# facebookresearch/brainmagick

Hardware: AMD Instinct MI355X
Metric: segments/s, 208-ch x 360-sample SimpleConv + ClipLoss training step (higher is better)
Workload: dtype f32 (fp32-accurate: operands split into 2 scaled f16 planes, 3 MFMA products, fp32 accumulate; same parity tolerances as exact fp32, see DESIGN.md §2); 1 GPU; cfg2: gwilliams2022-shaped MEG C=208 T=360, F=120 features, 27 subjects, clip_conv SimpleConv (8985590 params) + ClipLoss + Adam; batch_per_gpu=256, global_batch=256, negatives=local, parallelism=dp1, comm=none, rccl_world=1, candidate_gather=none, distinct_batches=8

## Files before the change

brainmagick_amd/csrc/core.hip:

```cpp
#include "bm_common.h"
#include <stdarg.h>
#include <stdlib.h>

thread_local char bm_err_buf[512] = {0};

int bm_set_error(int code, const char* fmt, ...) {
    va_list ap;
    va_start(ap, fmt);
    vsnprintf(bm_err_buf, sizeof(bm_err_buf), fmt, ap);
    va_end(ap);
    return code;
}

int bm_check_launch(const char* what) {
    hipError_t e = hipGetLastError();
    if (e != hipSuccess) return bm_set_error((int)e, "%s: launch failed: %s", what, hipGetErrorString(e));
    return BM_OK;
}

extern "C" const char* bm_last_error(void) { return bm_err_buf; }
extern "C" int bm_version(void) { return 108; }

extern "C" int bm_device_count(void) {
    int n = 0;
    hipError_t e = hipGetDeviceCount(&n);
    if (e != hipSuccess) { bm_set_error((int)e, "hipGetDeviceCount: %s", hipGetErrorString(e)); return -1; }
    return n;
}

__global__ __launch_bounds__(1024) void amax_finalize_kernel(const float* __restrict__ ws, int n, float* __restrict__ out) {
    __shared__ float sh[16];
    float m = 0.f;
    for (int i = threadIdx.x; i < n; i += 1024) m = fmaxf(m, ws[i]);
    m = bm_wave_max(m);
    if ((threadIdx.x & 63) == 0) sh[threadIdx.x >> 6] = m;
    __syncthreads();
    if (threadIdx.x < BM_AMAX_SHARDS) {
        float v = 0.f;
        if (threadIdx.x == 0)
            for (int w = 0; w < 16; ++w) v = fmaxf(v, sh[w]);
        out[threadIdx.x] = v;
    }
}

int bm_amax_finalize(const float* ws, int n, float* out, hipStream_t stream) {
    if (!out) return BM_OK;
    hipLaunchKernelGGL(amax_finalize_kernel, dim3(1), dim3(1024), 0, stream, ws, n, out);
    return bm_check_launch("amax_finalize");
}

__global__ __launch_bounds__(1024) void amax_finalize_rows_kernel(const float* __restrict__ ws, int C, int nsplit,
                                                                  float* __restrict__ out, float* __restrict__ rows_out,
                                                                  const double* __restrict__ sum_partial,
                                                                  float* __restrict__ sums_out) {
// ... 40 lines not shown
```

brainmagick_amd/csrc/norm_act.hip:

```cpp
#include <cstdlib>
#include "bm_common.h"

template <int VEC> struct Pack;
template <> struct Pack<1> {
    float v[1];
    __device__ static Pack ld(const float* p) { Pack r; r.v[0] = *p; return r; }
    __device__ void st(float* p) const { *p = v[0]; }
};
template <> struct Pack<4> {
    float v[4];
    __device__ static Pack ld(const float* p) {
        const float4 t = *reinterpret_cast<const float4*>(p);
        Pack r; r.v[0] = t.x; r.v[1] = t.y; r.v[2] = t.z; r.v[3] = t.w; return r;
    }
    __device__ void st(float* p) const { *reinterpret_cast<float4*>(p) = make_float4(v[0], v[1], v[2], v[3]); }
};

#define LAUNCH_VEC(vec4, kernel, grid, stream, ...)                                              \
    do {                                                                                         \
        if (vec4) hipLaunchKernelGGL(kernel<4>, grid, dim3(256), 0, stream, __VA_ARGS__);        \
        else hipLaunchKernelGGL(kernel<1>, grid, dim3(256), 0, stream, __VA_ARGS__);             \
    } while (0)
static int flat_blocks(long n) { return (int)((n + 255) / 256 > 16384 ? 16384 : (n + 255) / 256); }

// ... 577 lines not shown
    if (workspace_bytes < bm_channel_sum_workspace_bytes(B, C))
        return bm_set_error(BM_ERR_WORKSPACE, "channel_sum: workspace too small");
    hipStream_t s = (hipStream_t)stream;
    double* partial = (double*)workspace;
    LAUNCH_VEC(T % 4 == 0 && bstride % 4 == 0, channel_sum_kernel, dim3(C, nsplit), s, x, bstride, partial, B, C, T);
    hipLaunchKernelGGL(finalize_channel_sums_kernel, dim3(cdiv(C, 256)), dim3(256), 0, s, partial, out, C,
                       nsplit);
    return bm_check_launch("channel_sum");
}

__global__ __launch_bounds__(256) void time_sums_t_kernel(const float* __restrict__ x, float* __restrict__ out,
                                                          int B, int C, int T) {
    const long row = (long)blockIdx.x * 4 + (threadIdx.x >> 6);
    if (row >= (long)B * C) return;
    const int lane = threadIdx.x & 63;
    const float* p = x + row * T;
    float s = 0.f;
    for (int t = lane; t < T; t += 64) s += p[t];
    s = bm_wave_sum(s);
    if (lane == 0) {
        const int b = (int)(row / C), c = (int)(row - (long)b * C);
        out[(long)c * B + b] = s;
    }
}

extern "C" int bm_time_sums_t(const float* x, float* out, int B, int C, int T, void* stream) {
    BM_REQUIRE(x && out && B >= 0 && C > 0 && T > 0, "time_sums_t: bad arguments");
    if (B == 0) return BM_OK;
    hipLaunchKernelGGL(time_sums_t_kernel, dim3((unsigned)(((long)B * C + 3) / 4)), dim3(256), 0, (hipStream_t)stream,
                       x, out, B, C, T);
    return bm_check_launch("time_sums_t");
}

template <int VEC>
__global__ __launch_bounds__(256) void channel_stats_kernel(const float* __restrict__ x,
                                                            float* __restrict__ stats, int B, int C,
                                                            int T) {
    __shared__ double sh[4 * 2];
    const int c = blockIdx.x, split = blockIdx.y, nsplit = gridDim.y;
    const Slab sl(B, split, nsplit, T, VEC);
    float s = 0.f, s2 = 0.f;
    for (SlabWalk w(sl.TV, threadIdx.x, blockDim.x); w.bl < sl.nb; w.next()) {
        const int bl = w.bl, tv = w.tv;
        const Pack<VEC> v = Pack<VEC>::ld(x + ((long)(sl.b0 + bl) * C + c) * T + (long)tv * VEC);
#pragma unroll
        for (int i = 0; i < VEC; ++i) { s += v.v[i]; s2 += v.v[i] * v.v[i]; }
    }
    double acc[2] = {(double)s, (double)s2};
    block_sum<2>(acc, sh);
    if (threadIdx.x == 0) {
        stats[((long)split * C + c) * 2 + 0] = (float)acc[0];
        stats[((long)split * C + c) * 2 + 1] = (float)acc[1];
    }
}

extern "C" int bm_channel_stats_splits(int B) { return B >= 64 ? 16 : (B >= 8 ? 4 : 1); }

extern "C" int bm_channel_stats(const float* x, float* stats, int B, int C, int T, void* stream) {
    BM_REQUIRE(x && stats, "channel_stats: null pointer");
    const int nsplit = bm_channel_stats_splits(B);
    hipStream_t s = (hipStream_t)stream;
    LAUNCH_VEC(T % 4 == 0, channel_stats_kernel, dim3(C, nsplit), s, x, stats, B, C, T);
    return bm_check_launch("channel_stats");
}

template <int VEC>
// ... 109 lines not shown
```

brainmagick_amd/csrc/pack.hip:

```cpp
#include "bm_common.h"

__global__ void pack_weights_kernel(const float* __restrict__ src, float* __restrict__ dst, int G,
                                    int M, int Cin, int KS, long sg, long sm, long sc, long sj,
                                    int flip, int Mpad, int nchunk, const float* alpha_ptr) {
    const long total = (long)G * nchunk * KS * BM_BKC * Mpad;
    const float alpha = alpha_ptr ? *alpha_ptr : 1.f;
    for (long i = (long)blockIdx.x * blockDim.x + threadIdx.x; i < total;
         i += (long)gridDim.x * blockDim.x) {
        long r = i;
        const int m = (int)(r % Mpad); r /= Mpad;
        const int cc = (int)(r % BM_BKC); r /= BM_BKC;
        const int j = (int)(r % KS); r /= KS;
        const int chunk = (int)(r % nchunk);
        const int g = (int)(r / nchunk);
        const int c = chunk * BM_BKC + cc;
        float v = 0.f;
        if (m < M && c < Cin) {
            const int jj = flip ? KS - 1 - j : j;
            v = alpha * src[g * sg + m * sm + c * sc + jj * sj];
        }
        dst[i] = v;
    }
}

// ... 39 lines not shown
        int run = 0;
        for (int g = 0; g < G; ++g) { const int c = counts[g]; counts[g] = run; seg[g] = run; run += c; }
        counts[G] = run;
        seg[G] = run;
    }
    __syncthreads();
    for (int g = threadIdx.x; g < G; g += blockDim.x) {
        int pos = counts[g];
        const int end = counts[g + 1];
        for (int b0 = 0; b0 < B && pos < end; b0 += 8) {
            int v[8];
#pragma unroll
            for (int u = 0; u < 8; ++u) v[u] = b0 + u < B ? ids[b0 + u] : -1;
#pragma unroll
            for (int u = 0; u < 8; ++u)
                if (v[u] == g) order[pos++] = b0 + u;
        }
    }
}

#define BM_GROUP_MAX_INTS (64 * 1024 / 4)

extern "C" int bm_group_by_index(const long* idx, int B, int G, int* order, int* seg, int* err_flag,
                                 void* stream) {
    BM_REQUIRE(seg && ((idx && order) || B == 0), "group_by_index: null pointer");
    BM_REQUIRE(B >= 0 && G > 0, "group_by_index: bad dims B=%d G=%d", B, G);
    BM_REQUIRE((long)G + 1 + B <= BM_GROUP_MAX_INTS, "group_by_index: B + G + 1 = %ld ints of LDS exceed the %d of a "
               "launch (B=%d G=%d)", (long)G + 1 + B, BM_GROUP_MAX_INTS, B, G);
    hipLaunchKernelGGL(group_by_index_kernel, dim3(1), dim3(256), (size_t)(G + 1 + B) * sizeof(int),
                       (hipStream_t)stream, idx, B, G, order, seg, err_flag);
    return bm_check_launch("group_by_index");
}

__global__ void index_to_i32_kernel(const long* __restrict__ idx, int B, int G, int* __restrict__ out,
                                    int* __restrict__ err) {
    const int i = blockIdx.x * blockDim.x + threadIdx.x;
    if (i >= B) return;
    long v = idx[i];
    if (v < 0 || v >= G) {
        if (err) atomicExch(err, 1);
        v = 0;
    }
    out[i] = (int)v;
}

extern "C" int bm_index_to_i32(const long* idx, int B, int G, int* out, int* err_flag, void* stream) {
    BM_REQUIRE((idx && out) || B == 0, "index_to_i32: null pointer");
    BM_REQUIRE(B >= 0 && G > 0, "index_to_i32: bad dims B=%d G=%d", B, G);
    if (B == 0) return BM_OK;
    hipLaunchKernelGGL(index_to_i32_kernel, dim3((B + 255) / 256), dim3(256), 0, (hipStream_t)stream, idx, B,
                       G, out, err_flag);
    return bm_check_launch("index_to_i32");
}

__global__ void reduce_splits_kernel(const float* __restrict__ part, float* __restrict__ out, int G,
                                     int nsplit, int M, int Cn, int KS, long sg, long sm, long sc,
                                     long sj) {
    const long N = (long)Cn * KS;
    const long per = (long)M * N;
    const long total = (long)G * per;
    for (long i = (long)blockIdx.x * blockDim.x + threadIdx.x; i < total;
         i += (long)gridDim.x * blockDim.x) {
        const int g = (int)(i / per);
        const long r = i - (long)g * per;
        const int m = (int)(r / N);
        const int n = (int)(r - (long)m * N);
// ... 83 lines not shown
```

brainmagick_amd/functional.py:

```python

import torch

from . import hip_ops as H



ACT_CODES = {"none": H.ACT_NONE, "gelu": H.ACT_GELU, "relu": H.ACT_RELU, "leaky": H.ACT_LEAKY}


def _c(t: torch.Tensor) -> torch.Tensor:
    return t if t.is_contiguous() else t.contiguous()


_arange_cache = {}


def _arange_i32(n: int, device, repeat: int = 1) -> torch.Tensor:
    key = (n, repeat, device.type, device.index)
    t = _arange_cache.get(key)
    if t is None:
        if len(_arange_cache) > 64:
            _arange_cache.clear()
        t = torch.arange(n, dtype=torch.int32, device=device)
        if repeat != 1:
            t = t.repeat(repeat)
        if device.type == "cuda":
            torch.cuda.current_stream(device).synchronize()
        _arange_cache[key] = t
    return t


def _conv_weight_grads(dy, x, weight, KS, dil, transposed_weight):
    dst = H.grad_destination(weight)
    B, M, T = dy.shape
    Cin = x.shape[1]
    if transposed_weight:
        out = dst if dst is not None else torch.empty(weight.shape, device=dy.device, dtype=torch.float32)
        H.gemm_nt(x, dy, B, Cin, M, T, 1, 1, out=out.view(1, Cin, M, 1))
        return out.view(weight.shape) if dst is not None else out
    if dst is not None:
        H.gemm_nt(dy, x, B, M, Cin, T, KS, dil, out=dst.view(1, M, Cin, KS))
        return dst.view(weight.shape)
    return H.gemm_nt(dy, x, B, M, Cin, T, KS, dil).view(weight.shape)


def _layer_forward(x, weight, geom, res=None, **kw):
    dil, transposed, stride, pad = geom
    if pad is not None:
        assert res is None, "the strided family has no fused residual"
        KS = weight.shape[2]
        M = weight.shape[1] if transposed else weight.shape[0]
        Tout = H.conv_out_len(x.shape[2], KS, stride, dil, pad, transposed)
        wp = H.pack_strided_rows_second(weight) if transposed else H.pack_strided_rows_first(weight)
        return H.conv_strided(x, wp, M, Tout, KS, stride, dil, pad, transposed, **kw)
    assert stride == 1
    if transposed:
        Cin, M, KS = weight.shape
        assert KS == 1, "ConvTranspose1d is only supported with kernel 1 (simpleconv.py:189)"
# ... 185 lines not shown
        U, C, O, D = ctx.dims
        dout = _c(dout)
        B, _, T = meg.shape
        dheads = None
        if ctx.needs_input_grad[1]:
            order, seg = H.group_by_index(_c(layout_index.to(torch.int64)), U)
            dweights = H.gemm_nt(dout, meg, B, O, C, T, 1, 1, order=order, seg=seg, G=U).view(U, O, C)
            dscores = H.softmax_bwd(weights, dweights)
            wp = H.pack_weights(dscores, U, O, C, 1, O * C, C, 1, 0, shape=(D, 1))
            uidx = _arange_i32(U, meg.device)
            _, per_layout, _ = H.conv_nn(emb, wp, O, 1, 1, widx=uidx)
            if ctx.per_layout_heads:
                dheads = per_layout
            else:
                dheads = H.sum_over_batch(per_layout) if U > 1 else per_layout[0]
        dmeg = None
        if ctx.needs_input_grad[0]:
            wpt = H.pack_weights(weights, U, C, O, 1, O * C, 1, C, 0, shape=(T, 1))
            _, dmeg, _ = H.conv_nn(dout, wpt, C, 1, 1, widx=widx)
        return dmeg, dheads, None, None, None, None


class FusedFrontEndFn(torch.autograd.Function):

    @staticmethod
    def forward(ctx, meg, heads, w1, b1, ws, positions_u, layout_index, subjects, ban_center, ban_radius: float):
        meg, heads, w1, ws, positions_u = _c(meg), _c(heads), _c(w1), _c(ws), _c(positions_u)
        U, C, _ = positions_u.shape
        O, Dp = heads.shape
        L = w1.shape[0]
        S, _, D = ws.shape
        B, _, T = meg.shape
        dev = meg.device
        emb = H.fourier_emb(positions_u, Dp)
        seg_u = _arange_i32(U + 1, dev)
        scores = H.gemm_nt(heads, emb, U, O, C, Dp, a_strides=(0, Dp), x_strides=(C * Dp, Dp), seg=seg_u,
                           G=U).view(U, O, C)
        wm = H.masked_softmax(scores, positions_u, ban_center, ban_radius)
        _, p, _ = H.conv_nn(wm, H.pack_conv_fwd(w1), L, 1, 1)
        bcol = (b1 if b1 is not None else torch.zeros(L, device=dev)).view(1, L, 1).expand(U, L, 1)
        xp = torch.cat([p, bcol], dim=2).repeat_interleave(S, dim=0).contiguous()
        widx_p = _arange_i32(S, dev, repeat=U)
        _, wc, _ = H.conv_nn(xp, H.pack_weights(ws, S, D, L, 1, L * D, 1, D, 0), D, 1, 1, widx=widx_p)
        bias_c = wc[:, :, C].contiguous()
        pair = H.index_i32(_c(layout_index.to(torch.int64)), U) * S + H.index_i32(_c(subjects.to(torch.int64)), S)
        wpc = H.pack_weights(wc, U * S, D, C, 1, D * (C + 1), C + 1, 1, 0, shape=(T, 1))
        _, out, _ = H.conv_nn(meg, wpc, D, 1, 1, widx=pair, bias=bias_c, bias_gstride=D)
        ctx.save_for_backward(meg, emb, wm, xp, ws, w1, pair, widx_p, wc)
        ctx.dims = (U, C, O, Dp, L, S, D)
        ctx.has_b1 = b1 is not None
        return out

    @staticmethod
    def backward(ctx, dout):
        meg, emb, wm, xp, ws, w1, pair, widx_p, wc = ctx.saved_tensors
        U, C, O, Dp, L, S, D = ctx.dims
        dout = _c(dout)
        B, _, T = meg.shape
        dev = meg.device
        P = U * S
        order, seg = H.group_by_index(pair.to(torch.int64), P)
        gaug = torch.empty(P, D, C + 1, device=dev, dtype=torch.float32)
        H.gemm_nt(dout, meg, B, D, C, T, 1, 1, order=order, seg=seg, G=P, out=gaug,
                  out_strides=(D * (C + 1), C + 1, 1, 0))
        gaug[:, :, C] = H.segment_sum_cols(H.time_sums_t(dout), order, seg).t()
        seg_p = _arange_i32(P + 1, dev)
        dws = dw1 = db1 = dheads = None
        if ctx.needs_input_grad[4]:
            t1 = H.gemm_nt(xp, gaug, P, L, D, C + 1, seg=seg_p, G=P)
            dws = (H.sum_over_batch(t1.view(U, S * L * D)) if U > 1 else t1).view(S, L, D)
        _, a, _ = H.conv_nn(gaug, H.pack_weights(ws, S, L, D, 1, L * D, D, 1, 0), L, 1, 1, widx=widx_p)
        a_u = torch.stack([H.sum_over_batch(a[u * S:(u + 1) * S]) for u in range(U)])
        if ctx.has_b1 and ctx.needs_input_grad[3]:
            db1 = H.sum_over_batch(a_u[:, :, C].contiguous()) if U > 1 else a_u[0, :, C].contiguous()
        if ctx.needs_input_grad[2]:
            dw1 = H.gemm_nt(a_u, wm, U, L, O, C, 1, 1, a_strides=(L * (C + 1), C + 1),
                            x_strides=(O * C, C)).view(L, O, 1)
        if ctx.needs_input_grad[1]:
            _, dwm, _ = H.conv_nn(a_u, H.pack_conv_dgrad(w1), O, 1, 1)
            dscores = H.softmax_bwd(wm, dwm[:, :, :C].contiguous())
            wp = H.pack_weights(dscores, U, O, C, 1, O * C, C, 1, 0, shape=(Dp, 1))
            uidx = _arange_i32(U, dev)
            _, per_layout, _ = H.conv_nn(emb, wp, O, 1, 1, widx=uidx)
            dheads = H.sum_over_batch(per_layout) if U > 1 else per_layout[0]
        dmeg = None
        if ctx.needs_input_grad[0]:
            wpt = H.pack_weights(wc, P, C, D, 1, D * (C + 1), 1, C + 1, 0, shape=(T, 1))
            _, dmeg, _ = H.conv_nn(dout, wpt, C, 1, 1, widx=pair)
        return dmeg, dheads, dw1, db1, dws, None, None, None, None, None


_CLIP_BLOCK_BYTES = 0x3f000000


def _candidate_blocks(Bc: int, K: int):
    if Bc * K * 4 < _CLIP_BLOCK_BYTES:
        return [(0, Bc)]
    rows = max(1, _CLIP_BLOCK_BYTES // (K * 4))
    if rows >= 128:
        rows -= rows % 128
    return [(r0, min(rows, Bc - r0)) for r0 in range(0, Bc, rows)]


def _clip_raw_scores(estimate, candidate, B, Bc, K):
    blocks = _candidate_blocks(Bc, K)
    if len(blocks) == 1:
        return H.gemm_nt_partials(estimate, candidate, 1, B, Bc, K, (0, K), (0, K))
    raw = torch.empty(1, B, Bc, device=estimate.device, dtype=torch.float32)
    cand2 = candidate.view(Bc, K)
    for r0, rows in blocks:
        blk = H.share_amax(candidate, cand2[r0:r0 + rows])
        H.gemm_nt(estimate, blk, 1, B, rows, K, 1, 1, a_strides=(0, K), x_strides=(0, K),
                  out=raw.view(-1)[r0:], out_strides=(0, Bc, 1, 0))
    return raw


class ClipLossFn(torch.autograd.Function):

    @staticmethod
    def forward(ctx, estimate, candidate, target_offset: int = 0, col_valid=None, symmetric: bool = False,
# ... 180 lines not shown
```

brainmagick_amd/hip_ops.py:

```python
import ctypes
import typing as tp

import torch

from ._lib import lib, check, BmHipError

ACT_NONE, ACT_GELU, ACT_RELU, ACT_LEAKY = 0, 1, 2, 3
BKC = 16

import os as _os
DEFAULT_COMPUTE_DTYPE = "f16x2"
COMPUTE_DTYPES = ("f32", "f32x3", "f16x2")
_compute_dtype = _os.environ.get("BM_COMPUTE_DTYPE", DEFAULT_COMPUTE_DTYPE)
if _compute_dtype not in COMPUTE_DTYPES:
    raise ValueError(f"BM_COMPUTE_DTYPE must be one of {COMPUTE_DTYPES}, got {_compute_dtype!r}")


def set_compute_dtype(name: str):
    global _compute_dtype
    if name not in COMPUTE_DTYPES:
        raise ValueError(f"compute dtype must be one of {COMPUTE_DTYPES}, got {name!r}")
    _compute_dtype = name


# ... 653 lines not shown
                              _p(_opt(mean, "mean")), _p(_opt(invstd, "invstd")), int(bn_train),
                              _p(dy), _p(dgamma), _p(dbeta), _p(dbias), _p(ws), nbytes, B, C, T, act,
                              leak, *_slot_args(slot), _p(_row_amax_out(dy, slot)), _stream()), "bm_act_bn_bwd")
    return dy, dgamma, dbeta, dbias


def channel_sum(x: torch.Tensor) -> torch.Tensor:
    _req(x, "channel_sum.x")
    B, C, T = x.shape
    out = torch.empty(C, device=x.device, dtype=torch.float32)
    nbytes = lib().bm_channel_sum_workspace_bytes(B, C)
    ws = torch.empty(nbytes, device=x.device, dtype=torch.uint8)
    check(lib().bm_channel_sum(_p(x), C * T, _p(out), _p(ws), nbytes, B, C, T, _stream()),
          "bm_channel_sum")
    return out


def channel_stats(x: torch.Tensor) -> torch.Tensor:
    _req(x, "channel_stats.x")
    B, C, T = x.shape
    stats = torch.empty(lib().bm_channel_stats_splits(B), C, 2, device=x.device, dtype=torch.float32)
    check(lib().bm_channel_stats(_p(x), _p(stats), B, C, T, _stream()), "bm_channel_stats")
    return stats


def time_sums_t(x: torch.Tensor) -> torch.Tensor:
    _req(x, "time_sums_t.x")
    B, C, T = x.shape
    out = torch.empty(C, B, device=x.device, dtype=torch.float32)
    check(lib().bm_time_sums_t(_p(x), _p(out), B, C, T, _stream()), "bm_time_sums_t")
    return out


def glu_fwd(u: torch.Tensor) -> torch.Tensor:
    _req(u, "glu_fwd.u")
    B, C2, T = u.shape
    out = torch.empty(B, C2 // 2, T, device=u.device, dtype=torch.float32)
    check(lib().bm_glu_fwd(_p(u), _p(out), B, C2 // 2, T, *_slot_args(_amax_slot(out)), _stream()), "bm_glu_fwd")
    return out


def glu_bwd(dout: torch.Tensor, u: torch.Tensor, want_dbias: bool = True):
    _req(dout, "glu_bwd.dout")
    _req(u, "glu_bwd.u")
    B, C2, T = u.shape
    H = C2 // 2
    du = torch.empty_like(u)
    dbias = torch.empty(C2, device=u.device, dtype=torch.float32) if want_dbias else None
    nbytes = lib().bm_glu_bwd_workspace_bytes(B, H)
    ws = torch.empty(nbytes, device=u.device, dtype=torch.uint8)
    slot = _amax_slot(du)
    check(lib().bm_glu_bwd(_p(dout), _p(u), _p(du), _p(dbias), _p(ws), nbytes, B, H, T,
                           *_slot_args(slot), _p(_row_amax_out(du, slot)), _stream()), "bm_glu_bwd")
    return du, dbias


def fourier_emb(positions: torch.Tensor, D: int, margin: float = 0.2) -> torch.Tensor:
    _req(positions, "fourier_emb.positions")
    rows = positions.numel() // 2
    emb = torch.empty(*positions.shape[:-1], D, device=positions.device, dtype=torch.float32)
    check(lib().bm_fourier_emb(_p(positions), _p(emb), rows, D, margin, _stream()), "bm_fourier_emb")
    return emb


def masked_softmax(scores, positions, ban_center, ban_radius: float) -> torch.Tensor:
    _req(scores, "masked_softmax.scores")
# ... 360 lines not shown
```

include/bm_hip.h:

```cpp
#ifndef BM_HIP_H
#define BM_HIP_H
#ifdef __cplusplus
extern "C" {
#endif

#define BM_ACT_NONE 0
#define BM_ACT_GELU 1
#define BM_ACT_RELU 2
#define BM_ACT_LEAKY 3

int bm_version(void);
const char* bm_last_error(void);
int bm_device_count(void);

int bm_conv_mt_for(int M);
int bm_conv_mpad(int M);
int bm_conv_stats_tiles(int B, int T);
long bm_packed_weight_elems(int G, int M, int Cin, int KS);
int bm_pack_weights(const float* src, float* dst, int G, int M, int Cin, int KS, long sg, long sm,
                    long sc, long sj, int flip, const float* alpha_ptr, void* stream);
int bm_group_by_index(const long* idx, int B, int G, int* order, int* seg, int* err_flag, void* stream);
int bm_index_to_i32(const long* idx, int B, int G, int* out, int* err_flag, void* stream);
int bm_reduce_splits(const float* part, float* out, int G, int nsplit, int M, int Cn, int KS, long sg,
                     long sm, long sc, long sj, void* stream);
int bm_sum_over_batch(const float* x, float* out, int B, long n, void* stream);

int bm_conv1d_nn(const float* x, long x_bstride, const float* wpacked, const int* widx,
                 const float* bias, long bias_gstride, const float* ep_scale, const float* ep_shift, const float* res,
                 long res_bstride, float* y_pre, float* y_out, long y_bstride, float* stats, int B,
                 int Cin, int M, int T, int KS, int dil, int act, float leak, void* stream);

int bm_conv1d_out_len(int T, int KS, int stride, int dil, int pad, int transposed);
int bm_conv_strided_stats_tiles(int B, int Tout, int stride, int transposed);
int bm_conv1d_strided(const float* x, long x_bstride, const float* wpacked, const float* bias,
                      const float* ep_scale, const float* ep_shift, float* y_pre, float* y_out, long y_bstride,
                      float* stats, int B, int Cin, int M, int T, int Tout, int KS, int stride, int dil, int pad,
                      int act, float leak, void* stream);
int bm_conv1d_transposed(const float* x, long x_bstride, const float* wpacked, const float* bias,
                         const float* ep_scale, const float* ep_shift, float* y_pre, float* y_out, long y_bstride,
                         float* stats, int B, int Cin, int M, int T, int Tout, int KS, int stride, int dil, int pad,
                         int act, float leak, void* stream);
int bm_conv1d_strided_wgrad_suggest_splits(int R, int Q, int KS, int S, int U);
int bm_conv1d_strided_wgrad(const float* a, long a_sstride, const float* xl, long xl_sstride, float* part, int S,
                            int R, int Q, int U, int L, int KS, int stride, int dil, int pad, int nsplit,
                            void* stream);

int bm_lstm_layer_fwd(const float* whh0, const float* whh1, const float* gx0, const float* gx1, float* y,
                      float* gates0, float* gates1, float* c0, float* c1, int H, int B, int T, int dirs,
                      void* stream);
int bm_lstm_layer_bwd(const float* whh0, const float* whh1, const float* dy, const float* gates0,
                      const float* gates1, const float* c0, const float* c1, float* dg0, float* dg1,
                      float* dc0, float* dc1, int H, int B, int T, int dirs, void* stream);

long bm_packed_weight_elems_x3(int G, int M, int Cin, int KS);
int bm_pack_weights_x3(const float* src, void* dst, int G, int M, int Cin, int KS, long sg, long sm,
                       long sc, long sj, int flip, const float* alpha_ptr, void* stream);
int bm_conv1d_nn_x3(const float* x, long x_bstride, const void* wpacked, const int* widx,
                    const float* bias, long bias_gstride, const float* ep_scale, const float* ep_shift, const float* res,
// ... 56 lines not shown
                   void* stream);
int bm_bn_finalize_cm(const float* stats, int ntiles, int C, long count, const float* gamma,
                   const float* beta, float* running_mean, float* running_var, long* num_batches,
                   float momentum, float eps, float* mean, float* invstd, float* scale, float* shift,
                   void* stream);
int bm_bn_eval_affine(int C, const float* gamma, const float* beta, const float* running_mean,
                      const float* running_var, float eps, float* mean, float* invstd, float* scale,
                      float* shift, void* stream);
int bm_affine_act_res(const float* y, const float* scale, const float* shift, const float* res,
                      float* out, int B, int C, int T, int act, float leak, float* amax_out, float* amax_ws,
                      void* stream);
int bm_bwd_nsplit(int B);
long bm_act_bn_bwd_workspace_bytes(int B, int C);
int bm_act_bn_bwd_set_fused(int mode);
int bm_act_bn_bwd_set_poll_limit(int polls);
long bm_act_bn_bwd_fused_fallbacks(void);
int bm_act_bn_bwd_fused_covers(int B, int C, int T);
int bm_act_bn_bwd(const float* dout, const float* y, const float* scale, const float* shift,
                  const float* mean, const float* invstd, int bn_train, float* dy, float* dgamma,
                  float* dbeta, float* dbias, void* workspace, long workspace_bytes, int B, int C,
                  int T, int act, float leak, float* amax_out, float* amax_ws, float* amax_rows_out,
                  void* stream);
long bm_channel_sum_workspace_bytes(int B, int C);
int bm_channel_sum(const float* x, long bstride, float* out, void* workspace, long workspace_bytes,
                   int B, int C, int T, void* stream);
int bm_channel_stats_splits(int B);
int bm_channel_stats(const float* x, float* stats, int B, int C, int T, void* stream);
int bm_glu_fwd(const float* u, float* out, int B, int H, int T, float* amax_out, float* amax_ws, void* stream);
long bm_glu_bwd_workspace_bytes(int B, int H);
int bm_glu_bwd(const float* dout, const float* u, float* du, float* dbias, void* workspace,
               long workspace_bytes, int B, int H, int T, float* amax_out, float* amax_ws,
               float* amax_rows_out, void* stream);
int bm_time_sums_t(const float* x, float* out, int B, int C, int T, void* stream);

int bm_center_scale(const float* x, float* out, const long* group, const float* center,
                    const float* scale, int B, int C, int T, int clip, float limit, float* maxabs,
                    void* stream);

long bm_quantile_select_workspace_bytes(int C, int Q);
int bm_quantile_select(const float* x, const long* ranks, float* out, int N, int C, int T, int Q, void* workspace,
                       long workspace_bytes, void* stream);
long bm_masked_moments_workspace_bytes(int channels);
int bm_masked_moments(const float* x, const unsigned char* mask, int mask_mode, int N, int F, int T, int f0, int f1,
                      int per_channel, float* mean, float* std, double* count, void* workspace, long workspace_bytes,
                      void* stream);
long bm_category_counts_workspace_bytes(int cardinality);
int bm_category_counts(const float* x, const unsigned char* mask, int mask_mode, int N, int F, int T, int f,
                       int cardinality, float* counts, int* flags, void* workspace, long workspace_bytes, void* stream);
int bm_center_scale_inverse(const float* x, float* out, const long* group, const float* center, const float* scale,
                            int B, int C, int T, void* stream);

int bm_fourier_emb(const float* positions, float* emb, long rows, int D, float margin, void* stream);
int bm_masked_softmax(const float* scores, const float* positions, const float* ban_center,
                      float ban_radius, float* weights, int U, int O, int C, void* stream);
int bm_softmax_bwd(const float* w, const float* dw, float* ds, long rows, int C, void* stream);

int bm_clip_inv_norms(const float* cand, int Bc, long K, float* inv_norm, void* stream);
int bm_clip_cand_prep(const float* cand, int Bc, long K, float* inv_norm, float* amax_slot, int* nonfinite_flag,
                      void* stream);
int bm_flag_unless_all_set(const unsigned char* mask, long n, int* flag, void* stream);
int bm_clip_ce(const float* part, int nsplit, const float* inv_norm, float* scores, float* probs,
               float* dscaled, float* loss_row, float* loss, int B, int Bc, int target_offset,
               void* stream);
int bm_clip_ce_masked(const float* part, int nsplit, const float* inv_norm, const float* col_valid, float* scores,
                      float* probs, float* dscaled, float* loss_row, float* loss, int B, int Bc, int target_offset,
                      void* stream);
// ... 48 lines not shown
```

Measured before the change: 17390 segments/s.

## Replace conv-based spatial-attention and subject-layer algebra with a batched small-GEMM kernel

```diff
diff --git a/brainmagick_amd/csrc/core.hip b/brainmagick_amd/csrc/core.hip
--- a/brainmagick_amd/csrc/core.hip
+++ b/brainmagick_amd/csrc/core.hip
@@ -19,7 +19,7 @@
 }
 
 extern "C" const char* bm_last_error(void) { return bm_err_buf; }
-extern "C" int bm_version(void) { return 108; }
+extern "C" int bm_version(void) { return 109; }
 
 extern "C" int bm_device_count(void) {
     int n = 0;
diff --git a/brainmagick_amd/csrc/norm_act.hip b/brainmagick_amd/csrc/norm_act.hip
--- a/brainmagick_amd/csrc/norm_act.hip
+++ b/brainmagick_amd/csrc/norm_act.hip
@@ -633,6 +633,34 @@
     return bm_check_launch("time_sums_t");
 }
 
+__global__ __launch_bounds__(256) void group_time_sums_kernel(const float* __restrict__ x, const int* __restrict__ order,
+                                                              const int* __restrict__ seg, float* __restrict__ out,
+                                                              int B, int G, int C, int T, long sg, long sc) {
+    const long row = (long)blockIdx.x * 4 + (threadIdx.x >> 6);
+    if (row >= (long)G * C) return;
+    const int g = (int)(row / C), c = (int)(row - (long)g * C);
+    const int lane = threadIdx.x & 63;
+    const int k0 = max(seg[g], 0), k1 = min(seg[g + 1], B);
+    float s = 0.f;
+    for (int k = k0; k < k1; ++k) {
+        const int b = order[k];
+        if (b < 0 || b >= B) continue;
+        const float* p = x + ((long)b * C + c) * T;
+#pragma unroll 4
+        for (int t = lane; t < T; t += 64) s += p[t];
+    }
+    s = bm_wave_sum(s);
+    if (lane == 0) out[g * sg + c * sc] = s;
+}
+
+extern "C" int bm_group_time_sums(const float* x, const int* order, const int* seg, float* out, int B, int G, int C,
+                                  int T, long sg, long sc, void* stream) {
+    BM_REQUIRE(seg && out && ((x && order) || B == 0) && B >= 0 && G > 0 && C > 0 && T > 0, "group_time_sums: bad arguments");
+    hipLaunchKernelGGL(group_time_sums_kernel, dim3((unsigned)(((long)G * C + 3) / 4)), dim3(256), 0,
+                       (hipStream_t)stream, x, order, seg, out, B, G, C, T, sg, sc);
+    return bm_check_launch("group_time_sums");
+}
+
 template <int VEC>
 __global__ __launch_bounds__(256) void channel_stats_kernel(const float* __restrict__ x,
                                                             float* __restrict__ stats, int B, int C,
diff --git a/brainmagick_amd/csrc/pack.hip b/brainmagick_amd/csrc/pack.hip
--- a/brainmagick_amd/csrc/pack.hip
+++ b/brainmagick_amd/csrc/pack.hip
@@ -95,6 +95,57 @@
     return bm_check_launch("group_by_index");
 }
 
+__global__ void pair_group_kernel(const long* __restrict__ layout, const long* __restrict__ subject, int B, int U,
+                                  int S, int* __restrict__ pair, int* __restrict__ order, int* __restrict__ seg,
+                                  int* __restrict__ err) {
+    extern __shared__ int counts[];
+    const int G = U * S;
+    int* ids = counts + G + 1;
+    for (int g = threadIdx.x; g <= G; g += blockDim.x) counts[g] = 0;
+    __syncthreads();
+    for (int b = threadIdx.x; b < B; b += blockDim.x) {
+        long u = layout[b], s = subject[b];
+        if (u < 0 || u >= U) { if (err) atomicExch(err, 1); u = 0; }
+        if (s < 0 || s >= S) { if (err) atomicExch(err, 1); s = 0; }
+        const int p = (int)u * S + (int)s;
+        pair[b] = p;
+        ids[b] = p;
+        atomicAdd(&counts[p], 1);
+    }
+    __syncthreads();
+    if (threadIdx.x == 0) {
+        int run = 0;
+        for (int g = 0; g < G; ++g) { const int c = counts[g]; counts[g] = run; seg[g] = run; run += c; }
+        counts[G] = run;
+        seg[G] = run;
+    }
+    __syncthreads();
+    for (int g = threadIdx.x; g < G; g += blockDim.x) {
+        int pos = counts[g];
+        const int end = counts[g + 1];
+        for (int b0 = 0; b0 < B && pos < end; b0 += 8) {
+            int v[8];
+#pragma unroll
+            for (int u = 0; u < 8; ++u) v[u] = b0 + u < B ? ids[b0 + u] : -1;
+#pragma unroll
+            for (int u = 0; u < 8; ++u)
+                if (v[u] == g) order[pos++] = b0 + u;
+        }
+    }
+}
+
+extern "C" int bm_pair_group(const long* layout, const long* subject, int B, int U, int S, int* pair, int* order,
+                             int* seg, int* err_flag, void* stream) {
+    BM_REQUIRE(seg && ((layout && subject && pair && order) || B == 0), "pair_group: null pointer");
+    BM_REQUIRE(B >= 0 && U > 0 && S > 0 && (long)U * S <= BM_GROUP_MAX_INTS, "pair_group: bad dims B=%d U=%d S=%d", B, U, S);
+    const long G = (long)U * S;
+    BM_REQUIRE(G + 1 + B <= BM_GROUP_MAX_INTS, "pair_group: B + U * S + 1 = %ld ints of LDS exceed the %d of a launch",
+               G + 1 + B, BM_GROUP_MAX_INTS);
+    hipLaunchKernelGGL(pair_group_kernel, dim3(1), dim3(256), (size_t)(G + 1 + B) * sizeof(int), (hipStream_t)stream,
+                       layout, subject, B, U, S, pair, order, seg, err_flag);
+    return bm_check_launch("pair_group");
+}
+
 __global__ void index_to_i32_kernel(const long* __restrict__ idx, int B, int G, int* __restrict__ out,
                                     int* __restrict__ err) {
     const int i = blockIdx.x * blockDim.x + threadIdx.x;
diff --git a/brainmagick_amd/csrc/small_gemm.hip b/brainmagick_amd/csrc/small_gemm.hip
--- /dev/null
+++ b/brainmagick_amd/csrc/small_gemm.hip
@@ -0,0 +1,187 @@
+#include "bm_common.h"
+
+extern "C" int bm_reduce_splits(const float* part, float* out, int G, int nsplit, int M, int Cn, int KS, long sg,
+                                long sm, long sc, long sj, void* stream);
+
+#define SG_T 32
+#define SG_KC 64
+#define SG_LD 33
+#define SG_THREADS 256
+#define SG_PER (SG_T * SG_KC / SG_THREADS)
+
+struct SmallGemmArgs {
+    const float* A;
+    const float* B;
+    float* out;
+    float* part;
+    const int* gidx;
+    const float* col;
+    float* last_col;
+    int M, N, K, R, G, GA, GB;
+    int nsplit, stages_per_r, stages_per_split;
+    int extra_col;
+    long sag, sar, sam, sak;
+    long sbg, sbr, sbk, sbn;
+    long scg, scm, scn;
+};
+
+__global__ __launch_bounds__(SG_THREADS) void small_gemm_kernel(const SmallGemmArgs a) {
+    __shared__ float smem[2 * 2 * SG_KC * SG_LD];
+    const int tid = threadIdx.x;
+    const int lane = tid & 63, wave = tid >> 6;
+    const int tiles_n = (a.N + SG_T - 1) / SG_T;
+    const int m0 = (blockIdx.x / tiles_n) * SG_T;
+    const int n0 = (blockIdx.x % tiles_n) * SG_T;
+    const int split = blockIdx.y;
+    const int g = blockIdx.z;
+    int ga = g, gb = g;
+    if (a.gidx) {
+        ga = min(max(a.gidx[2 * g], 0), a.GA - 1);
+        gb = min(max(a.gidx[2 * g + 1], 0), a.GB - 1);
+    }
+    const float* Ag = a.A + ga * a.sag;
+    const float* Bg = a.B + gb * a.sbg;
+
+    const bool a_kfast = a.sak == 1;
+    const bool b_kfast = a.sbk == 1 && a.sbn != 1;
+    float ra[SG_PER], rb[SG_PER];
+    int ao[SG_PER], bo[SG_PER], akk[SG_PER], bkk[SG_PER];
+    short al[SG_PER], bl[SG_PER];
+#pragma unroll
+    for (int i = 0; i < SG_PER; ++i) {
+        const int e = i * SG_THREADS + tid;
+        int x, kk;
+        if (a_kfast) { kk = e % SG_KC; x = e / SG_KC; } else { x = e % SG_T; kk = e / SG_T; }
+        akk[i] = m0 + x < a.M ? kk : a.K;
+        ao[i] = (int)((m0 + x) * a.sam + kk * a.sak);
+        al[i] = (short)(kk * SG_LD + x);
+        if (b_kfast) { kk = e % SG_KC; x = e / SG_KC; } else { x = e % SG_T; kk = e / SG_T; }
+        bkk[i] = n0 + x < a.N ? kk : a.K;
+        bo[i] = (int)(kk * a.sbk + (n0 + x) * a.sbn);
+        bl[i] = (short)(kk * SG_LD + x);
+    }
+
+    const int total_stages = a.R * a.stages_per_r;
+    const int s_begin = split * a.stages_per_split;
+    const int s_end = min(s_begin + a.stages_per_split, total_stages);
+
+#define SG_LOAD(s)                                                                                       \
+    {                                                                                                    \
+        const int r_ = (s) / a.stages_per_r;                                                             \
+        const int k0_ = ((s) - r_ * a.stages_per_r) * SG_KC;                                             \
+        const float* Ar = Ag + r_ * a.sar + k0_ * a.sak;                                                 \
+        const float* Br = Bg + r_ * a.sbr + k0_ * a.sbk;                                                 \
+        const int krem = a.K - k0_;                                                                      \
+        _Pragma("unroll") for (int i = 0; i < SG_PER; ++i) {                                             \
+            ra[i] = akk[i] < krem ? Ar[ao[i]] : 0.f;                                                     \
+            rb[i] = bkk[i] < krem ? Br[bo[i]] : 0.f;                                                     \
+        }                                                                                                \
+    }
+#define SG_STORE(buf)                                                                                    \
+    {                                                                                                    \
+        float* As_ = smem + (buf) * 2 * SG_KC * SG_LD;                                                   \
+        float* Bs_ = As_ + SG_KC * SG_LD;                                                                \
+        _Pragma("unroll") for (int i = 0; i < SG_PER; ++i) {                                             \
+            As_[al[i]] = ra[i];                                                                          \
+            Bs_[bl[i]] = rb[i];                                                                          \
+        }                                                                                                \
+    }
+
+    f32x16 acc;
+#pragma unroll
+    for (int i = 0; i < 16; ++i) acc[i] = 0.f;
+
+    if (s_begin < s_end) {
+        SG_LOAD(s_begin);
+        SG_STORE(0);
+    }
+    __syncthreads();
+    for (int s = s_begin; s < s_end; ++s) {
+        const int buf = (s - s_begin) & 1;
+        const bool more = s + 1 < s_end;
+        if (more) SG_LOAD(s + 1);
+        const float* ap = smem + buf * 2 * SG_KC * SG_LD + (wave * (SG_KC / 4) + (lane >> 5)) * SG_LD + (lane & 31);
+        const float* bp = ap + SG_KC * SG_LD;
+#pragma unroll
+        for (int p = 0; p < SG_KC / 8; ++p)
+            acc = __builtin_amdgcn_mfma_f32_32x32x2f32(ap[2 * p * SG_LD], bp[2 * p * SG_LD], acc, 0, 0, 0);
+        if (more) SG_STORE(buf ^ 1);
+        __syncthreads();
+    }
+#undef SG_LOAD
+#undef SG_STORE
+
+    float* red = smem + wave * SG_T * SG_LD;
+#pragma unroll
+    for (int i = 0; i < 16; ++i)
+        red[((i >> 2) * 8 + (lane >> 5) * 4 + (i & 3)) * SG_LD + (lane & 31)] = acc[i];
+    __syncthreads();
+    const bool to_part = a.nsplit > 1;
+    float* dst = to_part ? a.part + ((long)g * a.nsplit + split) * a.M * a.N : a.out + g * a.scg;
+    const long dm = to_part ? a.N : a.scm, dn = to_part ? 1 : a.scn;
+#pragma unroll
+    for (int i = 0; i < SG_T * SG_T / SG_THREADS; ++i) {
+        const int e = i * SG_THREADS + tid;
+        const int row = e / SG_T, c = e % SG_T;
+        const float* q = smem + row * SG_LD + c;
+        const float v = ((q[0] + q[SG_T * SG_LD]) + q[2 * SG_T * SG_LD]) + q[3 * SG_T * SG_LD];
+        if (m0 + row < a.M && n0 + c < a.N) {
+            dst[(long)(m0 + row) * dm + (long)(n0 + c) * dn] = v;
+            if (a.last_col && n0 + c == a.N - 1) a.last_col[(long)g * a.M + m0 + row] = v;
+        }
+    }
+    if (a.extra_col && n0 == 0 && split == 0 && tid < SG_T && m0 + tid < a.M)
+        a.out[g * a.scg + (long)(m0 + tid) * a.scm + (long)a.N * a.scn] = a.col ? a.col[m0 + tid] : 0.f;
+}
+
+extern "C" int bm_small_gemm_suggest_splits(int M, int N, int K, int R, int G) {
+    if (M <= 0 || N <= 0 || K <= 0 || R <= 0 || G <= 0) return 1;
+    const long tiles = (long)cdiv(M, SG_T) * cdiv(N, SG_T) * G;
+    const long stages = (long)R * cdiv(K, SG_KC);
+    if (stages <= 8) return 1;
+    long n = (1024 + tiles - 1) / tiles;
+    if (n > stages / 4) n = stages / 4;
+    if (n > 32) n = 32;
+    if (n < 1) n = 1;
+    const long per = (stages + n - 1) / n;
+    return (int)((stages + per - 1) / per);
+}
+
+extern "C" long bm_small_gemm_part_elems(int M, int N, int G, int nsplit) {
+    return nsplit > 1 ? (long)G * nsplit * M * N : 0;
+}
+
+extern "C" int bm_small_gemm(const float* A, long sag, long sar, long sam, long sak, const float* B, long sbg,
+                             long sbr, long sbk, long sbn, float* out, long scg, long scm, long scn,
+                             const int* gidx, int GA, int GB, const float* col, int extra_col, float* last_col,
+                             float* part, int G, int R, int M, int N, int K, int nsplit, void* stream) {
+    BM_REQUIRE(A && B && out, "small_gemm: null pointer");
+    BM_REQUIRE(G > 0 && R > 0 && M > 0 && N > 0 && K > 0, "small_gemm: bad dims G=%d R=%d M=%d N=%d K=%d", G, R, M, N, K);
+    BM_REQUIRE(G <= 65535, "small_gemm: G=%d exceeds the grid's z extent", G);
+    BM_REQUIRE(min(min(sam, sak), min(sbk, sbn)) >= 0 && (M + 31L) * sam + (K + 63L) * sak < 0x7fffffffL &&
+               (K + 63L) * sbk + (N + 31L) * sbn < 0x7fffffffL, "small_gemm: a matrix must span less than 2^31 elements");
+    BM_REQUIRE(!gidx || (GA > 0 && GB > 0), "small_gemm: an index table needs the group counts of A and B");
+    BM_REQUIRE(!col || extra_col, "small_gemm: a column vector without extra_col");
+    const int stages_per_r = cdiv(K, SG_KC);
+    const long stages = (long)R * stages_per_r;
+    BM_REQUIRE(nsplit >= 1 && nsplit <= 65535, "small_gemm: nsplit=%d outside [1, 65535]", nsplit);
+    if (nsplit > stages) nsplit = (int)stages;
+    BM_REQUIRE(nsplit == 1 || part, "small_gemm: nsplit > 1 needs the partial-tile workspace");
+    BM_REQUIRE(nsplit == 1 || !last_col, "small_gemm: the copy of the last column needs nsplit == 1");
+    SmallGemmArgs a;
+    a.A = A; a.B = B; a.out = out; a.part = part; a.gidx = gidx; a.col = col; a.last_col = last_col;
+    a.M = M; a.N = N; a.K = K; a.R = R; a.G = G; a.GA = GA; a.GB = GB;
+    a.stages_per_r = stages_per_r;
+    a.stages_per_split = cdiv(stages, nsplit);
+    a.nsplit = cdiv(stages, a.stages_per_split);
+    a.extra_col = extra_col;
+    a.sag = sag; a.sar = sar; a.sam = sam; a.sak = sak;
+    a.sbg = sbg; a.sbr = sbr; a.sbk = sbk; a.sbn = sbn;
+    a.scg = scg; a.scm = scm; a.scn = scn;
+    const long tiles = (long)cdiv(M, SG_T) * cdiv(N, SG_T);
+    BM_REQUIRE(tiles <= 0x7fffffffL, "small_gemm: too many tiles");
+    hipLaunchKernelGGL(small_gemm_kernel, dim3((unsigned)tiles, a.nsplit, G), dim3(SG_THREADS), 0, (hipStream_t)stream, a);
+    const int rc = bm_check_launch("small_gemm");
+    if (rc != BM_OK || a.nsplit == 1) return rc;
+    return bm_reduce_splits(part, out, G, a.nsplit, M, N, 1, scg, scm, scn, 0, stream);
+}
diff --git a/brainmagick_amd/functional.py b/brainmagick_amd/functional.py
--- a/brainmagick_amd/functional.py
+++ b/brainmagick_amd/functional.py
@@ -24,6 +24,20 @@
         t = torch.arange(n, dtype=torch.int32, device=device)
         if repeat != 1:
             t = t.repeat(repeat)
+        if device.type == "cuda":
+            torch.cuda.current_stream(device).synchronize()
+        _arange_cache[key] = t
+    return t
+
+
+def _pair_table(U: int, S: int, device) -> torch.Tensor:
+    key = ("pair", U, S, device.type, device.index)
+    t = _arange_cache.get(key)
+    if t is None:
+        if len(_arange_cache) > 64:
+            _arange_cache.clear()
+        p = torch.arange(U * S, dtype=torch.int32)
+        t = torch.stack([p % S, p // S], dim=1).contiguous().to(device)
         if device.type == "cuda":
             torch.cuda.current_stream(device).synchronize()
         _arange_cache[key] = t
@@ -275,60 +289,67 @@
         S, _, D = ws.shape
         B, _, T = meg.shape
         dev = meg.device
+        C1 = C + 1
         emb = H.fourier_emb(positions_u, Dp)
         seg_u = _arange_i32(U + 1, dev)
         scores = H.gemm_nt(heads, emb, U, O, C, Dp, a_strides=(0, Dp), x_strides=(C * Dp, Dp), seg=seg_u,
                            G=U).view(U, O, C)
         wm = H.masked_softmax(scores, positions_u, ban_center, ban_radius)
-        _, p, _ = H.conv_nn(wm, H.pack_conv_fwd(w1), L, 1, 1)
-        bcol = (b1 if b1 is not None else torch.zeros(L, device=dev)).view(1, L, 1).expand(U, L, 1)
-        xp = torch.cat([p, bcol], dim=2).repeat_interleave(S, dim=0).contiguous()
-        widx_p = _arange_i32(S, dev, repeat=U)
-        _, wc, _ = H.conv_nn(xp, H.pack_weights(ws, S, D, L, 1, L * D, 1, D, 0), D, 1, 1, widx=widx_p)
-        bias_c = wc[:, :, C].contiguous()
-        pair = H.index_i32(_c(layout_index.to(torch.int64)), U) * S + H.index_i32(_c(subjects.to(torch.int64)), S)
-        wpc = H.pack_weights(wc, U * S, D, C, 1, D * (C + 1), C + 1, 1, 0, shape=(T, 1))
+        paug = torch.empty(U, L, C1, device=dev, dtype=torch.float32)
+        H.small_gemm(w1, (0, 0, O, 1), wm, (O * C, 0, C, 1), paug, (L * C1, C1, 1), U, 1, L, C, O,
+                     col=_c(b1) if b1 is not None else None, extra_col=True)
+        wc = torch.empty(U * S, D, C1, device=dev, dtype=torch.float32)
+        bias_c = torch.empty(U * S, D, device=dev, dtype=torch.float32)
+        H.small_gemm(ws, (L * D, 0, 1, D), paug, (L * C1, 0, C1, 1), wc, (D * C1, C1, 1), U * S, 1, D, C1, L,
+                     gidx=_pair_table(U, S, dev), groups=(S, U), last_col=bias_c)
+        pair, order, seg = H.pair_group(_c(layout_index.to(torch.int64)), _c(subjects.to(torch.int64)), U, S)
+        wpc = H.pack_weights(wc, U * S, D, C, 1, D * C1, C1, 1, 0, shape=(T, 1))
         _, out, _ = H.conv_nn(meg, wpc, D, 1, 1, widx=pair, bias=bias_c, bias_gstride=D)
-        ctx.save_for_backward(meg, emb, wm, xp, ws, w1, pair, widx_p, wc)
+        ctx.save_for_backward(meg, emb, wm, paug, ws, w1, pair, order, seg, wc, heads)
         ctx.dims = (U, C, O, Dp, L, S, D)
         ctx.has_b1 = b1 is not None
         return out
 
     @staticmethod
     def backward(ctx, dout):
-        meg, emb, wm, xp, ws, w1, pair, widx_p, wc = ctx.saved_tensors
+        meg, emb, wm, paug, ws, w1, pair, order, seg, wc, heads = ctx.saved_tensors
         U, C, O, Dp, L, S, D = ctx.dims
         dout = _c(dout)
         B, _, T = meg.shape
         dev = meg.device
         P = U * S
-        order, seg = H.group_by_index(pair.to(torch.int64), P)
-        gaug = torch.empty(P, D, C + 1, device=dev, dtype=torch.float32)
+        C1 = C + 1
+
+        def grad_out(param, shape):
+            dst = H.grad_destination(param)
+            return dst if dst is not None else torch.empty(shape, device=dev, dtype=torch.float32)
+        gaug = torch.empty(P, D, C1, device=dev, dtype=torch.float32)
         H.gemm_nt(dout, meg, B, D, C, T, 1, 1, order=order, seg=seg, G=P, out=gaug,
-                  out_strides=(D * (C + 1), C + 1, 1, 0))
-        gaug[:, :, C] = H.segment_sum_cols(H.time_sums_t(dout), order, seg).t()
-        seg_p = _arange_i32(P + 1, dev)
+                  out_strides=(D * C1, C1, 1, 0))
+        H.group_time_sums(dout, order, seg, gaug.view(-1)[C:], (D * C1, C1))
         dws = dw1 = db1 = dheads = None
         if ctx.needs_input_grad[4]:
-            t1 = H.gemm_nt(xp, gaug, P, L, D, C + 1, seg=seg_p, G=P)
-            dws = (H.sum_over_batch(t1.view(U, S * L * D)) if U > 1 else t1).view(S, L, D)
-        _, a, _ = H.conv_nn(gaug, H.pack_weights(ws, S, L, D, 1, L * D, D, 1, 0), L, 1, 1, widx=widx_p)
-        a_u = torch.stack([H.sum_over_batch(a[u * S:(u + 1) * S]) for u in range(U)])
+            dws = grad_out(ws, ws.shape)
+            H.small_gemm(paug, (0, L * C1, C1, 1), gaug, (D * C1, S * D * C1, 1, C1), dws, (L * D, D, 1), S, U, L, D, C1)
+            dws = dws.view(ws.shape)
+        a_u = torch.empty(U, L, C1, device=dev, dtype=torch.float32)
+        H.small_gemm(ws, (0, L * D, D, 1), gaug, (S * D * C1, D * C1, C1, 1), a_u, (L * C1, C1, 1), U, S, L, C1, D)
         if ctx.has_b1 and ctx.needs_input_grad[3]:
             db1 = H.sum_over_batch(a_u[:, :, C].contiguous()) if U > 1 else a_u[0, :, C].contiguous()
         if ctx.needs_input_grad[2]:
-            dw1 = H.gemm_nt(a_u, wm, U, L, O, C, 1, 1, a_strides=(L * (C + 1), C + 1),
-                            x_strides=(O * C, C)).view(L, O, 1)
+            dw1 = grad_out(w1, w1.shape)
+            H.small_gemm(a_u, (0, L * C1, C1, 1), wm, (0, O * C, 1, C), dw1, (0, O, 1), 1, U, L, O, C)
+            dw1 = dw1.view(L, O, 1)
         if ctx.needs_input_grad[1]:
-            _, dwm, _ = H.conv_nn(a_u, H.pack_conv_dgrad(w1), O, 1, 1)
-            dscores = H.softmax_bwd(wm, dwm[:, :, :C].contiguous())
-            wp = H.pack_weights(dscores, U, O, C, 1, O * C, C, 1, 0, shape=(Dp, 1))
-            uidx = _arange_i32(U, dev)
-            _, per_layout, _ = H.conv_nn(emb, wp, O, 1, 1, widx=uidx)
-            dheads = H.sum_over_batch(per_layout) if U > 1 else per_layout[0]
+            dwm = torch.empty(U, O, C, device=dev, dtype=torch.float32)
+            H.small_gemm(w1, (0, 0, 1, O), a_u, (L * C1, 0, C1, 1), dwm, (O * C, C, 1), U, 1, O, C, L)
+            dscores = H.softmax_bwd(wm, dwm)
+            dheads = grad_out(heads, (O, Dp))
+            H.small_gemm(dscores, (0, O * C, C, 1), emb, (0, C * Dp, Dp, 1), dheads, (0, Dp, 1), 1, U, O, Dp, C)
+            dheads = dheads.view(O, Dp)
         dmeg = None
         if ctx.needs_input_grad[0]:
-            wpt = H.pack_weights(wc, P, C, D, 1, D * (C + 1), 1, C + 1, 0, shape=(T, 1))
+            wpt = H.pack_weights(wc, P, C, D, 1, D * C1, 1, C1, 0, shape=(T, 1))
             _, dmeg, _ = H.conv_nn(dout, wpt, C, 1, 1, widx=pair)
         return dmeg, dheads, dw1, db1, dws, None, None, None, None, None
 
diff --git a/brainmagick_amd/hip_ops.py b/brainmagick_amd/hip_ops.py
--- a/brainmagick_amd/hip_ops.py
+++ b/brainmagick_amd/hip_ops.py
@@ -709,6 +709,77 @@
     return out
 
 
+def group_time_sums(x: torch.Tensor, order: torch.Tensor, seg: torch.Tensor, out: torch.Tensor, out_strides) -> None:
+    _req(x, "group_time_sums.x")
+    _req(out, "group_time_sums.out")
+    B, C, T = x.shape
+    G = seg.numel() - 1
+    sg, sc = out_strides
+    if order.numel() != B or (G - 1) * sg + (C - 1) * sc >= out.numel() or min(sg, sc) < 0:
+        raise BmHipError("group_time_sums: order / output strides do not fit the tensors")
+    check(lib().bm_group_time_sums(_p(x), _p(_req(order, "order", torch.int32)), _p(_req(seg, "seg", torch.int32)),
+                                   _p(out), B, G, C, T, sg, sc, _stream()), "bm_group_time_sums")
+
+
+def pair_group(layout_index: torch.Tensor, subjects: torch.Tensor, U: int, S: int):
+    _req(layout_index, "pair_group.layout_index", torch.int64)
+    _req(subjects, "pair_group.subjects", torch.int64)
+    B = layout_index.numel()
+    if subjects.numel() != B:
+        raise BmHipError("pair_group: one layout and one subject index per segment")
+    dev = layout_index.device
+    pair = torch.empty(B, device=dev, dtype=torch.int32)
+    order = torch.empty(B, device=dev, dtype=torch.int32)
+    seg = torch.empty(U * S + 1, device=dev, dtype=torch.int32)
+    check(lib().bm_pair_group(_p(layout_index), _p(subjects), B, U, S, _p(pair), _p(order), _p(seg),
+                              _p(index_error_flag(dev)), _stream()), "bm_pair_group")
+    if _CHECK_INDICES_NOW:
+        raise_if_index_error(dev)
+    return pair, order, seg
+
+
+def small_gemm(a: torch.Tensor, a_strides, b: torch.Tensor, b_strides, out: torch.Tensor, out_strides, G: int, R: int,
+               M: int, N: int, K: int, gidx: tp.Optional[torch.Tensor] = None, groups=None,
+               col: tp.Optional[torch.Tensor] = None, extra_col: bool = False,
+               last_col: tp.Optional[torch.Tensor] = None, nsplit: tp.Optional[int] = None):
+    _req(a, "small_gemm.a")
+    _req(b, "small_gemm.b")
+    _req(out, "small_gemm.out")
+    GA, GB = groups if gidx is not None else (G, G)
+    if gidx is not None:
+        _req(gidx, "small_gemm.gidx", torch.int32)
+        if gidx.numel() != 2 * G:
+            raise BmHipError("small_gemm: gidx must be [G, 2]")
+    if col is not None:
+        _req(col, "small_gemm.col")
+        if not extra_col or col.numel() < M:
+            raise BmHipError("small_gemm: col needs extra_col and M elements")
+    sag, sar, sam, sak = a_strides
+    sbg, sbr, sbk, sbn = b_strides
+    scg, scm, scn = out_strides
+    if min(*a_strides, *b_strides, *out_strides) < 0 or min(G, R, M, N, K) < 1 or \
+            (GA - 1) * sag + (R - 1) * sar + (M - 1) * sam + (K - 1) * sak >= a.numel() or \
+            (GB - 1) * sbg + (R - 1) * sbr + (K - 1) * sbk + (N - 1) * sbn >= b.numel() or \
+            (G - 1) * scg + (M - 1) * scm + (N - 1 + int(extra_col)) * scn >= out.numel():
+        raise BmHipError(f"small_gemm: dims G={G} R={R} M={M} N={N} K={K} with strides {a_strides} {b_strides} "
+                         f"{out_strides} reach outside the tensors ({a.numel()}, {b.numel()}, {out.numel()} elements)")
+    if last_col is not None:
+        _req(last_col, "small_gemm.last_col")
+        if last_col.numel() != G * M:
+            raise BmHipError("small_gemm: last_col must be [G, M]")
+    if nsplit is None:
+        nsplit = 1 if last_col is not None else lib().bm_small_gemm_suggest_splits(M, N, K, R, G)
+    part = torch.empty(lib().bm_small_gemm_part_elems(M, N, G, nsplit), device=a.device, dtype=torch.float32) \
+        if nsplit > 1 else None
+
+    def launch():
+        check(lib().bm_small_gemm(_p(a), sag, sar, sam, sak, _p(b), sbg, sbr, sbk, sbn, _p(out), scg, scm, scn,
+                                  _p(gidx), GA, GB, _p(col), int(extra_col), _p(last_col), _p(part), G, R, M, N, K, nsplit,
+                                  _stream()), "bm_small_gemm")
+    _timed("small_gemm_kernel", 2.0 * G * R * M * N * K, launch)
+    return out
+
+
 def glu_fwd(u: torch.Tensor) -> torch.Tensor:
     _req(u, "glu_fwd.u")
     B, C2, T = u.shape
diff --git a/include/bm_hip.h b/include/bm_hip.h
--- a/include/bm_hip.h
+++ b/include/bm_hip.h
@@ -21,9 +21,18 @@
                     long sc, long sj, int flip, const float* alpha_ptr, void* stream);
 int bm_group_by_index(const long* idx, int B, int G, int* order, int* seg, int* err_flag, void* stream);
 int bm_index_to_i32(const long* idx, int B, int G, int* out, int* err_flag, void* stream);
+int bm_pair_group(const long* layout, const long* subject, int B, int U, int S, int* pair, int* order, int* seg,
+                  int* err_flag, void* stream);
 int bm_reduce_splits(const float* part, float* out, int G, int nsplit, int M, int Cn, int KS, long sg,
                      long sm, long sc, long sj, void* stream);
 int bm_sum_over_batch(const float* x, float* out, int B, long n, void* stream);
+
+int bm_small_gemm_suggest_splits(int M, int N, int K, int R, int G);
+long bm_small_gemm_part_elems(int M, int N, int G, int nsplit);
+int bm_small_gemm(const float* A, long sag, long sar, long sam, long sak, const float* B, long sbg, long sbr,
+                  long sbk, long sbn, float* out, long scg, long scm, long scn, const int* gidx, int GA, int GB,
+                  const float* col, int extra_col, float* last_col, float* part, int G, int R, int M, int N, int K,
+                  int nsplit, void* stream);
 
 int bm_conv1d_nn(const float* x, long x_bstride, const float* wpacked, const int* widx,
                  const float* bias, long bias_gstride, const float* ep_scale, const float* ep_shift, const float* res,
@@ -146,6 +155,8 @@
                long workspace_bytes, int B, int H, int T, float* amax_out, float* amax_ws,
                float* amax_rows_out, void* stream);
 int bm_time_sums_t(const float* x, float* out, int B, int C, int T, void* stream);
+int bm_group_time_sums(const float* x, const int* order, const int* seg, float* out, int B, int G, int C, int T,
+                       long sg, long sc, void* stream);
 
 int bm_center_scale(const float* x, float* out, const long* group, const float* center,
                     const float* scale, int B, int C, int T, int clip, float limit, float* maxabs,
```

Result: no change. 17220 segments/s (-1.0%).
